# quartiq/stabilizer-stream

Hardware: NVIDIA B200
Metric: sustained MS/s through full PSD cascade (higher is better)
Workload: dtype f32

## Files before the change

stabilizer_stream_b200/csrc/sspsd_cascade.cu:

```cuda
#if defined(__x86_64__)
#include <emmintrin.h>
#endif

#include "sspsd_cascade.cuh"

#include <algorithm>
#include <cmath>
#include <cstdlib>
#include <cstring>
#include <mutex>

#include "sspsd_decim_kernel.cuh"
#include "sspsd_stage_kernel.cuh"
#include "sspsd_stage_kernel_r16.cuh"
#include "sspsd_stage_kernel_ring.cuh"
#include "sspsd_stage_kernel_w16.cuh"

namespace sspsd {

static thread_local std::string g_err;
void set_error(const std::string& msg) { g_err = msg; }
const char* last_error() { return g_err.c_str(); }

bool cuda_ok(cudaError_t e, const char* what)
{
    if (e == cudaSuccess)
        return true;
    set_error(std::string(what) + ": " + cudaGetErrorString(e));
    return false;
}

namespace {

inline long long floor4(long long v) { return v & ~3ll; }

template <int LOG2N>
int launch_stage_t(const StageParams& p, int grid, cudaStream_t s)
{
    size_t smem = stage_smem_bytes<LOG2N>(p.T, p.hop);
    psd_stage_kernel<LOG2N><<<grid, Plan<LOG2N>::NT, smem, s>>>(p);
    return cuda_ok(cudaGetLastError(), "psd_stage_kernel launch") ? SSPSD_OK : SSPSD_ECUDA;
}

template <int LOG2N>
int prepare_stage_t(int hop, int budget_bytes, int* tmax)
{
    using PL = Plan<LOG2N>;
    int t = 256;
    while (t > 1 && (long long)stage_smem_bytes<LOG2N>(t, hop) > budget_bytes)
        --t;
    if ((long long)stage_smem_bytes<LOG2N>(t, hop) > budget_bytes) {
        set_error("FFT size does not fit in shared memory");
        return SSPSD_EINVAL;
    }
    *tmax = t;
    (void)PL::N;
    if (!cuda_ok(cudaFuncSetAttribute(psd_stage_kernel<LOG2N>, cudaFuncAttributeMaxDynamicSharedMemorySize,
// ... 27 lines not shown
    default:
        return SSPSD_EINVAL;
    }
}

int prepare_stage(int log2n, bool r16, int hop, int* tmax, int* nt)
{
    if (log2n == 12 && r16) {
        int t = 64;
        while (t > 1 && (long long)stage_r16_smem_bytes(t, hop) > 112 * 1024) --t;
        *tmax = t;
        *nt = R16::NT;
        SSPSD_CUDA(cudaFuncSetAttribute(psd_stage_kernel_r16, cudaFuncAttributeMaxDynamicSharedMemorySize,
                                        (int)stage_r16_smem_bytes(t, hop)));
        SSPSD_CUDA(cudaFuncSetAttribute(psd_stage_kernel_ring, cudaFuncAttributeMaxDynamicSharedMemorySize,
                                        (int)stage_ring_smem_bytes(RingCfg::MAX_W)));
        SSPSD_CUDA(cudaFuncSetAttribute(psd_stage_kernel_ring1, cudaFuncAttributeMaxDynamicSharedMemorySize,
                                        (int)stage_ring_smem_bytes(1024, 1, RingCfg::RING1, false)));
        SSPSD_CUDA(cudaFuncSetAttribute(psd_stage_kernel_ring1x5, cudaFuncAttributeMaxDynamicSharedMemorySize,
                                        (int)stage_ring_smem_bytes(384, 1, 3, false)));
        return SSPSD_OK;
    }
    if (log2n == 9)
        SSPSD_CUDA(cudaFuncSetAttribute(psd_stage_kernel_w16, cudaFuncAttributeMaxDynamicSharedMemorySize,
                                        (int)stage_w16_smem_bytes(W16::MAX_T)));
    switch (log2n) {
#define X(L)                                                                   \
    case L:                                                                    \
        *nt = Plan<L>::NT;                                                     \
        return prepare_stage_t<L>(hop, Plan<L>::NT <= 256 ? 100 * 1024 : 200 * 1024, tmax);
        SSPSD_FOR_SIZES(X)
#undef X
    default:
        set_error("n_fft must be a power of two in 64..8192");
        return SSPSD_EINVAL;
    }
}

template <int MA, int MB, int MC, int PRESET>
int launch_decim_t(const DecimParams& p, int grid, cudaStream_t s)
{
    using GE = DecGeom<MA, MB, MC>;
    decim8_kernel<MA, MB, MC, PRESET><<<grid, DEC_NT, GE::SMEM_FLOATS * sizeof(float), s>>>(p);
    return cuda_ok(cudaGetLastError(), "decim8_kernel launch") ? SSPSD_OK : SSPSD_ECUDA;
}

template <int MA, int MB, int MC, int PRESET, int OB, int CTAS>
int launch_decim_tma_t(const DecimParams& p, long long n_out, int num_sms, cudaStream_t s)
{
    const int ntiles = (int)((n_out + OB - 1) / OB);
    const int grid = std::min(ntiles, num_sms * CTAS);
    decim8_tma_kernel<MA, MB, MC, PRESET, OB, CTAS><<<grid, DEC_NT, decim_tma_smem_bytes<MA, MB, MC, OB>(), s>>>(p, ntiles);
    return cuda_ok(cudaGetLastError(), "decim8_tma_kernel launch") ? SSPSD_OK : SSPSD_ECUDA;
}

template <int MA, int MB, int MC, int PRESET, int OB, int CTAS>
int launch_decim_async_t(const DecimParams& p, long long n_out, int num_sms, cudaStream_t s)
{
    const int ntiles = (int)((n_out + OB - 1) / OB);
    const int grid = std::min(ntiles, num_sms * CTAS);
    decim8_async_kernel<MA, MB, MC, PRESET, OB, CTAS><<<grid, DEC_NT, decim_async_smem_bytes<MA, MB, MC, OB>(), s>>>(p, ntiles);
    return cuda_ok(cudaGetLastError(), "decim8_async_kernel launch") ? SSPSD_OK : SSPSD_ECUDA;
}

template <int MA, int MB, int MC, int PRESET, int OB, int CTAS>
int launch_decim_pf_t(const DecimParams& p, long long n_out, int num_sms, cudaStream_t s)
{
    const int ntiles = (int)((n_out + OB - 1) / OB);
    const int grid = std::min(ntiles, num_sms * CTAS);
    decim8_pf_kernel<MA, MB, MC, PRESET, OB, CTAS><<<grid, DEC_NT, decim_pf_smem_bytes<MA, MB, MC, OB>(), s>>>(p, ntiles);
    return cuda_ok(cudaGetLastError(), "decim8_pf_kernel launch") ? SSPSD_OK : SSPSD_ECUDA;
}

int decim_halo(int preset)
{
    return preset == SSPSD_HBF_98 ? DecGeom<3, 6, 15>::HALO : DecGeom<5, 10, 23>::HALO;
}

int upload_taps_once(int device)
{
    static std::mutex mu;
    static bool done[64] = {false};
    std::lock_guard<std::mutex> lock(mu);
    if (device < 64 && done[device])
        return SSPSD_OK;
    static_assert(sizeof(sspsd_hbf_taps) == sizeof(float) * SSPSD_HBF_NPRESET * 3 * SSPSD_HBF_MAXTAPS, "tap table");
    {
        float t0[SSPSD_HBF_NPRESET][3][SSPSD_HBF_MAXTAPS + 1], t1[SSPSD_HBF_NPRESET][3][SSPSD_HBF_MAXTAPS + 1];
        for (int p = 0; p < SSPSD_HBF_NPRESET; ++p)
            for (int s = 0; s < 3; ++s)
                for (int i = 0; i <= SSPSD_HBF_MAXTAPS; ++i) {
                    t0[p][s][i] = i < SSPSD_HBF_MAXTAPS ? sspsd_hbf_taps[p][s][i] : 0.f;
                    t1[p][s][i] = i + 1 < SSPSD_HBF_MAXTAPS ? sspsd_hbf_taps[p][s][i + 1] : 0.f;
                }
        SSPSD_CUDA(cudaMemcpyToSymbol(c_hbf_taps, t0, sizeof(t0)));
        SSPSD_CUDA(cudaMemcpyToSymbol(c_hbf_taps_sh, t1, sizeof(t1)));
    }
    SSPSD_CUDA(cudaFuncSetAttribute(decim8_kernel<5, 10, 23, SSPSD_HBF_140>, cudaFuncAttributeMaxDynamicSharedMemorySize,
                                    (int)(DecGeom<5, 10, 23>::SMEM_FLOATS * sizeof(float))));
    SSPSD_CUDA(cudaFuncSetAttribute(decim8_kernel<3, 6, 15, SSPSD_HBF_98>, cudaFuncAttributeMaxDynamicSharedMemorySize,
                                    (int)(DecGeom<3, 6, 15>::SMEM_FLOATS * sizeof(float))));
    SSPSD_CUDA(cudaFuncSetAttribute(decim8_async_kernel<5, 10, 23, SSPSD_HBF_140, 960, 2>,
                                    cudaFuncAttributeMaxDynamicSharedMemorySize, (int)decim_async_smem_bytes<5, 10, 23, 960>()));
    SSPSD_CUDA(cudaFuncSetAttribute(decim8_async_kernel<5, 10, 23, SSPSD_HBF_140, 640, 3>,
                                    cudaFuncAttributeMaxDynamicSharedMemorySize, (int)decim_async_smem_bytes<5, 10, 23, 640>()));
    SSPSD_CUDA(cudaFuncSetAttribute(decim8_async_kernel<3, 6, 15, SSPSD_HBF_98, 960, 2>,
                                    cudaFuncAttributeMaxDynamicSharedMemorySize, (int)decim_async_smem_bytes<3, 6, 15, 960>()));
    SSPSD_CUDA(cudaFuncSetAttribute(decim8_async_kernel<3, 6, 15, SSPSD_HBF_98, 640, 3>,
                                    cudaFuncAttributeMaxDynamicSharedMemorySize, (int)decim_async_smem_bytes<3, 6, 15, 640>()));
    SSPSD_CUDA(cudaFuncSetAttribute(decim8_tma_kernel<5, 10, 23, SSPSD_HBF_140, 960, 2>,
                                    cudaFuncAttributeMaxDynamicSharedMemorySize, (int)decim_tma_smem_bytes<5, 10, 23, 960>()));
    SSPSD_CUDA(cudaFuncSetAttribute(decim8_tma_kernel<5, 10, 23, SSPSD_HBF_140, 640, 3>,
                                    cudaFuncAttributeMaxDynamicSharedMemorySize, (int)decim_tma_smem_bytes<5, 10, 23, 640>()));
    SSPSD_CUDA(cudaFuncSetAttribute(decim8_tma_kernel<3, 6, 15, SSPSD_HBF_98, 960, 2>,
                                    cudaFuncAttributeMaxDynamicSharedMemorySize, (int)decim_tma_smem_bytes<3, 6, 15, 960>()));
    SSPSD_CUDA(cudaFuncSetAttribute(decim8_tma_kernel<3, 6, 15, SSPSD_HBF_98, 640, 3>,
                                    cudaFuncAttributeMaxDynamicSharedMemorySize, (int)decim_tma_smem_bytes<3, 6, 15, 640>()));
    SSPSD_CUDA(cudaFuncSetAttribute(decim8_tma_kernel<5, 10, 23, SSPSD_HBF_140, 768, 3>,
                                    cudaFuncAttributeMaxDynamicSharedMemorySize, (int)decim_tma_smem_bytes<5, 10, 23, 768>()));
    SSPSD_CUDA(cudaFuncSetAttribute(decim8_tma_kernel<3, 6, 15, SSPSD_HBF_98, 768, 3>,
                                    cudaFuncAttributeMaxDynamicSharedMemorySize, (int)decim_tma_smem_bytes<3, 6, 15, 768>()));
    SSPSD_CUDA(cudaFuncSetAttribute(decim8_pf_kernel<5, 10, 23, SSPSD_HBF_140, 960, 2>,
                                    cudaFuncAttributeMaxDynamicSharedMemorySize, (int)decim_pf_smem_bytes<5, 10, 23, 960>()));
    SSPSD_CUDA(cudaFuncSetAttribute(decim8_pf_kernel<5, 10, 23, SSPSD_HBF_140, 640, 3>,
                                    cudaFuncAttributeMaxDynamicSharedMemorySize, (int)decim_pf_smem_bytes<5, 10, 23, 640>()));
    SSPSD_CUDA(cudaFuncSetAttribute(decim8_pf_kernel<3, 6, 15, SSPSD_HBF_98, 960, 2>,
                                    cudaFuncAttributeMaxDynamicSharedMemorySize, (int)decim_pf_smem_bytes<3, 6, 15, 960>()));
    SSPSD_CUDA(cudaFuncSetAttribute(decim8_pf_kernel<3, 6, 15, SSPSD_HBF_98, 640, 3>,
                                    cudaFuncAttributeMaxDynamicSharedMemorySize, (int)decim_pf_smem_bytes<3, 6, 15, 640>()));
    if (device < 64)
        done[device] = true;
    return SSPSD_OK;
}

struct EwmaPlan {
    int jb;
    float g_first;
    float g_s;
    float total;
    uint32_t count_after;
};

EwmaPlan ewma_plan(uint32_t count, uint32_t avg, uint64_t S)
{
    EwmaPlan e{};
    uint32_t steady = avg + 1u;
    e.g_s = (float)avg / (float)steady;
    uint64_t jb;
    if (count > avg) {
        jb = 0;
        e.g_first = (float)avg / (float)count;
    } else {
        jb = (uint64_t)avg - count + 1;
        e.g_first = e.g_s;
    }
    if (jb >= S) {
        e.jb = (int)S;
        e.total = 1.0f;
        e.count_after = (uint32_t)(count + S);
    } else {
        e.jb = (int)jb;
        double t = (double)e.g_first;
        uint64_t n_s = S - 1 - jb;
        if (n_s > 0)
            t *= std::pow((double)e.g_s, (double)n_s);
        e.total = (float)t;
        e.count_after = steady;
    }
    return e;
}

}

int hbf_info(int hbf, uint32_t* drain, uint32_t* halo)
// ... 81 lines not shown
    std::vector<float> win(n);
    if (cfg.window == SSPSD_WINDOW_RECT) {
        std::fill(win.begin(), win.end(), 1.0f);
        win_ = {1.0f, 1.0f, 0};
    } else {
        const float pi = 3.14159265358979323846f;
        float df = pi / (float)n;
        for (uint32_t i = 0; i < n; ++i) {
            float s = sinf(df * (float)i);
            win[i] = s * s;
        }
        win_ = {0.25f, 1.5f, n / 2};
    }
    hop_ = n - win_.overlap;
    drain_ = sspsd_hbf_drain[cfg.hbf];
    int halo = decim_halo(cfg.hbf);
    hb_ = std::max<int>((int)win_.overlap, halo);
    hb_ = (hb_ + 7) & ~7;

    SSPSD_CUDA(cudaDeviceGetAttribute(&num_sms_, cudaDevAttrMultiProcessorCount, cfg.device));
    if (cfg.stream) {
        stream_ = (cudaStream_t)cfg.stream;
    } else {
        SSPSD_CUDA(cudaStreamCreateWithFlags(&stream_, cudaStreamNonBlocking));
        own_stream_ = true;
    }
    SSPSD_CUDA(cudaStreamCreateWithFlags(&copy_stream_, cudaStreamNonBlocking));
    const char* ov = getenv("SSPSD_OVERLAP");
    deep_from_ = ov ? (size_t)atoi(ov) : 1;
    if (max_stages_ > 1 && deep_from_ > 0 && !one_stream_) {
        int lo_prio = 0, hi_prio = 0;
        SSPSD_CUDA(cudaDeviceGetStreamPriorityRange(&lo_prio, &hi_prio));
        SSPSD_CUDA(cudaStreamCreateWithPriority(&deep_stream_, cudaStreamNonBlocking, hi_prio));
        SSPSD_CUDA(cudaEventCreateWithFlags(&ev_stage0_, cudaEventDisableTiming));
        SSPSD_CUDA(cudaEventCreateWithFlags(&ev_deep_, cudaEventDisableTiming));
        const char* ps = getenv("SSPSD_PSD_STREAM");
        if (!ps || atoi(ps) != 0) {
            SSPSD_CUDA(cudaStreamCreateWithPriority(&psd_stream_, cudaStreamNonBlocking, hi_prio));
            SSPSD_CUDA(cudaEventCreateWithFlags(&ev_psd_join_, cudaEventDisableTiming));
        }
    }
    for (int i = 0; i < 2; ++i) {
        SSPSD_CUDA(cudaEventCreateWithFlags(&ev_copied_[i], cudaEventDisableTiming));
        SSPSD_CUDA(cudaEventCreateWithFlags(&ev_free_[i], cudaEventDisableTiming));
        SSPSD_CUDA(cudaEventCreateWithFlags(&ev_stage_[i], cudaEventDisableTiming));
    }
    int rc = upload_taps_once(cfg.device);
    if (rc) return rc;
    defer_ = cfg_.deep_defer ? cfg_.deep_defer : (1ull << 26);
    if (const char* e = getenv("SSPSD_DEFER")) defer_ = strtoull(e, nullptr, 0);
    k2_variant_ = k2_variant_from_env();
    {
        const char* e = getenv("SSPSD_K3");
        std::string m = e ? e : "tma960";
        k3_variant_ = m == "tiled" ? 0 : m == "tma960" ? 1 : m == "tma640" ? 2 : m == "async640" ? 4 : m == "pf960" ? 5 :
                      m == "pf640" ? 6 : m == "tma768" ? 7 : 3;
    }
    rc = prepare_stage((int)log2n_, k2_variant_ >= 1, (int)hop_, &tmax_, &nt_);
    if (rc) return rc;

    const uint32_t m = n / 2;
    std::vector<float2> twM(m), twN(m);
    for (uint32_t k = 0; k < m; ++k) {
        double a = -2.0 * M_PI * (double)k / (double)m;
        twM[k] = make_float2((float)std::cos(a), (float)std::sin(a));
        double b = -2.0 * M_PI * (double)k / (double)n;
        twN[k] = make_float2((float)std::cos(b), (float)std::sin(b));
    }
    acc_stride_ = (m + 1 + 63) & ~63u;
    SSPSD_CUDA(cudaMalloc(&d_win_, n * sizeof(float)));
    SSPSD_CUDA(cudaMalloc(&d_twM_, m * sizeof(float2)));
    SSPSD_CUDA(cudaMalloc(&d_twN_, m * sizeof(float2)));
    SSPSD_CUDA(cudaMalloc(&d_acc_, (size_t)SSPSD_MAX_STAGES * acc_stride_ * sizeof(float)));
    SSPSD_CUDA(cudaMemcpyAsync(d_win_, win.data(), n * sizeof(float), cudaMemcpyHostToDevice, stream_));
    SSPSD_CUDA(cudaMemcpyAsync(d_twM_, twM.data(), m * sizeof(float2), cudaMemcpyHostToDevice, stream_));
    SSPSD_CUDA(cudaMemcpyAsync(d_twN_, twN.data(), m * sizeof(float2), cudaMemcpyHostToDevice, stream_));
    SSPSD_CUDA(cudaMemsetAsync(d_acc_, 0, (size_t)SSPSD_MAX_STAGES * acc_stride_ * sizeof(float), stream_));
    SSPSD_CUDA(cudaMallocHost(&h_acc_, (size_t)SSPSD_MAX_STAGES * acc_stride_ * sizeof(float)));
    SSPSD_CUDA(cudaStreamSynchronize(stream_));
    stages_.reserve(SSPSD_MAX_STAGES);
    n_ = n;
    return SSPSD_OK;
}

uint32_t Cascade::stage_avg(size_t i) const
{
    unsigned sh = (unsigned)(SSPSD_DEPTH * i);
    uint32_t v = sh >= 32 ? 0u : (avg_.count >> sh);
    return std::min(v, avg_.limit);
}

int Cascade::add_stage()
{
    if (stages_.size() >= SSPSD_MAX_STAGES) {
        set_error("too many stages");
        return SSPSD_EINVAL;
    }
    StageState st;
    const size_t cap = (size_t)hb_ + n_ + 16;
    cudaStream_t ss = stage_stream(stages_.size());
    if (!spare_.empty()) {
        StageState old = spare_.back();
        spare_.pop_back();
        st.carry[0] = old.carry[0];
        st.carry[1] = old.carry[1];
        st.fresh[0] = old.fresh[0];
        st.fresh[1] = old.fresh[1];
        st.fresh_cap = old.fresh_cap;
        st.ev_read[0] = old.ev_read[0];
// ... 149 lines not shown
    rc = launch_stage((int)log2n_, k2_variant_ >= 1, p, grid, psd_stream(i));
    prof_end(psd_stream(i));
    if (rc) return rc;
    return reduce_partials(i, grid * groups, p);
}

int Cascade::prepare_partials(size_t i, int rows, StageParams* p)
{
    p->part = nullptr;
    p->part_stride = 0;
    if (!(cfg_.flags & SSPSD_FLAG_DETERMINISTIC)) return SSPSD_OK;
    const int which = psd_stream(i) == stream_ ? 0 : 1;
    const size_t need = (size_t)rows * acc_stride_;
    if (need > part_cap_[which]) {
        SSPSD_CUDA(cudaStreamSynchronize(psd_stream(i)));
        if (d_part_[which]) SSPSD_CUDA(cudaFree(d_part_[which]));
        d_part_[which] = nullptr;
        SSPSD_CUDA(cudaMalloc(&d_part_[which], need * sizeof(float)));
        part_cap_[which] = need;
    }
    p->part = d_part_[which];
    p->part_stride = (int)acc_stride_;
    return SSPSD_OK;
}

int Cascade::reduce_partials(size_t i, int rows, const StageParams& p)
{
    if (!p.part) return SSPSD_OK;
    const int nb = (int)(n_ / 2 + 1);
    prof_begin(SSPSD_PROF_OTHER, 0, psd_stream(i));
    reduce_partials_kernel<<<(nb + 127) / 128, 128, 0, psd_stream(i)>>>(p.acc, p.part, rows, p.part_stride, nb);
    prof_end(psd_stream(i));
    return cuda_ok(cudaGetLastError(), "reduce_partials_kernel launch") ? SSPSD_OK : SSPSD_ECUDA;
}

int Cascade::launch_decim(size_t i, const StreamSrc& src, uint64_t m0, uint64_t m1, float* out_fresh,
                          long long out_split, long long out_cap)
{
    DecimParams p{};
    p.src = src;
    p.m0 = (long long)m0;
    p.m1 = (long long)m1;
    p.drain = drain_;
    p.out_fresh = out_fresh;
    p.out_split = out_split;
    p.out_cap = out_cap;
    p.preset = cfg_.hbf;
    long long lo = std::max<long long>(p.m0, p.drain);
    if (p.m1 <= lo)
        return SSPSD_OK;
    int grid = (int)((p.m1 - lo + DEC_OB - 1) / DEC_OB);
    cudaStream_t ss = stage_stream(i);
    static const bool fuse_carry = !getenv("SSPSD_CARRY_KERNEL");
    if (cc_valid_ && fuse_carry && (k3_variant_ == 1 || k3_variant_ == 2 || k3_variant_ == 7)) {
        p.cc = cc_pending_;
        cc_valid_ = false;
    }
    prof_begin(i == 0 ? SSPSD_PROF_DECIM_STAGE0 : SSPSD_PROF_DECIM_DEEP, (uint64_t)(p.m1 - lo) * 8, ss);
    int rc;
    if (k3_variant_ == 0) {
        rc = cfg_.hbf == SSPSD_HBF_98 ? launch_decim_t<3, 6, 15, SSPSD_HBF_98>(p, grid, ss)
                                      : launch_decim_t<5, 10, 23, SSPSD_HBF_140>(p, grid, ss);
    } else if (k3_variant_ == 1) {
        rc = cfg_.hbf == SSPSD_HBF_98 ? launch_decim_tma_t<3, 6, 15, SSPSD_HBF_98, 960, 2>(p, p.m1 - lo, num_sms_, ss)
                                      : launch_decim_tma_t<5, 10, 23, SSPSD_HBF_140, 960, 2>(p, p.m1 - lo, num_sms_, ss);
    } else if (k3_variant_ == 2) {
        rc = cfg_.hbf == SSPSD_HBF_98 ? launch_decim_tma_t<3, 6, 15, SSPSD_HBF_98, 640, 3>(p, p.m1 - lo, num_sms_, ss)
                                      : launch_decim_tma_t<5, 10, 23, SSPSD_HBF_140, 640, 3>(p, p.m1 - lo, num_sms_, ss);
    } else if (k3_variant_ == 3) {
        rc = cfg_.hbf == SSPSD_HBF_98 ? launch_decim_async_t<3, 6, 15, SSPSD_HBF_98, 960, 2>(p, p.m1 - lo, num_sms_, ss)
                                      : launch_decim_async_t<5, 10, 23, SSPSD_HBF_140, 960, 2>(p, p.m1 - lo, num_sms_, ss);
    } else if (k3_variant_ == 7) {
        rc = cfg_.hbf == SSPSD_HBF_98 ? launch_decim_tma_t<3, 6, 15, SSPSD_HBF_98, 768, 3>(p, p.m1 - lo, num_sms_, ss)
                                      : launch_decim_tma_t<5, 10, 23, SSPSD_HBF_140, 768, 3>(p, p.m1 - lo, num_sms_, ss);
    } else if (k3_variant_ == 5) {
        rc = cfg_.hbf == SSPSD_HBF_98 ? launch_decim_pf_t<3, 6, 15, SSPSD_HBF_98, 960, 2>(p, p.m1 - lo, num_sms_, ss)
                                      : launch_decim_pf_t<5, 10, 23, SSPSD_HBF_140, 960, 2>(p, p.m1 - lo, num_sms_, ss);
    } else if (k3_variant_ == 6) {
        rc = cfg_.hbf == SSPSD_HBF_98 ? launch_decim_pf_t<3, 6, 15, SSPSD_HBF_98, 640, 3>(p, p.m1 - lo, num_sms_, ss)
                                      : launch_decim_pf_t<5, 10, 23, SSPSD_HBF_140, 640, 3>(p, p.m1 - lo, num_sms_, ss);
    } else {
        rc = cfg_.hbf == SSPSD_HBF_98 ? launch_decim_async_t<3, 6, 15, SSPSD_HBF_98, 640, 3>(p, p.m1 - lo, num_sms_, ss)
                                      : launch_decim_async_t<5, 10, 23, SSPSD_HBF_140, 640, 3>(p, p.m1 - lo, num_sms_, ss);
    }
    prof_end(ss);
    return rc;
}

int Cascade::run_stage(size_t i, const float* fresh, long long split, uint64_t n_new)
{
    StageState& st = stages_[i];
    cudaStream_t ss = stage_stream(i);
    cudaStream_t ps = psd_stream(i);
    const uint64_t L1 = st.L + n_new;
    const uint64_t craw0 = st.craw;
    const uint64_t craw1 = L1 < n_ ? 0 : 1 + (L1 - n_) / hop_;
    const StreamSrc src{st.carry[st.cur], fresh, st.carry_start, split, (long long)L1};
    int rc;
    bool psd_launched = false;
    if (ps != ss && craw1 > craw0) {
        SSPSD_CUDA(cudaEventRecord(st.ev_in, ss));
        SSPSD_CUDA(cudaStreamWaitEvent(ps, st.ev_in, 0));
    }

    if (windowed_ && i < n_local_ && craw1 > craw0) {
        const uint64_t step = (uint64_t)hop_ << (SSPSD_DEPTH * i);
        const uint64_t c = own_offset(i);
        auto first_at_or_after = [&](uint64_t pos) { return pos <= c ? 0ull : (pos - c + step - 1) / step; };
        uint64_t klo = std::max<uint64_t>(first_at_or_after(own_lo_), (st.valid_from + hop_ - 1) / hop_);
        uint64_t khi = own_hi_ == ~0ull ? ~0ull : first_at_or_after(own_hi_);
        uint64_t a = std::max(craw0, klo), b = std::min(craw1, khi);
        if (b > a) {
            if (st.avg == 0xffffffffu) {
// ... 958 lines not shown
```

stabilizer_stream_b200/csrc/sspsd_cascade.cuh:

```cuda
#pragma once
#include <cuda_runtime.h>

#include <cstdint>
#include <string>
#include <vector>

#include "../../include/sspsd.h"
#include "sspsd_device.cuh"

namespace sspsd {

struct StageParams;
void set_error(const std::string& msg);
const char* last_error();
int hbf_info(int hbf, uint32_t* drain, uint32_t* halo);
bool cuda_ok(cudaError_t e, const char* what);

struct DeviceGuard {
    int prev = -1;
    bool ok = true;
    explicit DeviceGuard(int dev)
    {
        if (cudaGetDevice(&prev) != cudaSuccess) prev = -1;
        ok = prev == dev || cuda_ok(cudaSetDevice(dev), "cudaSetDevice");
// ... 98 lines not shown
    cudaStream_t stage_stream(size_t i) const { return (i < deep_from_ || !deep_stream_) ? stream_ : deep_stream_; }
    cudaStream_t psd_stream(size_t i) const { return (i >= deep_from_ && psd_stream_) ? psd_stream_ : stage_stream(i); }
    int join_streams();
    uint64_t defer_threshold(size_t j) const;
    int run_pending(size_t j);
    int flush_deferred();
    int ensure_fresh(StageState& st, size_t need, size_t reserve = 0);
    int ensure_in_buffers(size_t need);
    int process_host(const float* x, size_t n);
    int flush_staged();
    int feed_device_chunk(const float* x, size_t n);
    int feed_host_chunk(const float* xh, size_t n);
    static uint64_t host_chunk() { return 1ull << 23; }
    float gain_of(uint32_t count) const;
    uint32_t stage_avg(size_t i) const;
    uint64_t decimated(const StageState& st) const { return st.craw ? n_ + (st.craw - 1) * (uint64_t)hop_ : 0; }

    struct ProfRec {
        int cls;
        cudaEvent_t a, b;
        uint64_t units;
    };
    bool prof_on_ = false;
    std::vector<ProfRec> prof_;
    uint64_t launches_[SSPSD_PROF_NCLASS] = {0, 0, 0, 0, 0};
    void prof_begin(int cls, uint64_t units, cudaStream_t s);
    void prof_end(cudaStream_t s);

    bool windowed_ = false;
    uint64_t own_lo_ = 0, own_hi_ = ~0ull;
    uint32_t n_local_ = SSPSD_MAX_STAGES;
    float* d_tail_ = nullptr;
    size_t tail_cap_ = 0, tail_len_ = 0;
    uint64_t tail_first_ = 0;
    uint64_t seek_pos_ = 0;
    uint64_t next_valid_from(uint64_t valid) const;
    uint64_t own_offset(size_t i) const;

    StageHook* hook_ = nullptr;
    bool one_stream_ = false;
    sspsd_config cfg_{};
    uint32_t n_ = 0, log2n_ = 0, hop_ = 0, max_stages_ = SSPSD_MAX_STAGES;
    WindowInfo win_{};
    int detrend_ = 0;
    sspsd_avg_opts avg_{0xffffffffu, 0xffffffffu};
    int hb_ = 0;
    int drain_ = 0;
    int num_sms_ = 148;
    int tmax_ = 1, nt_ = 256;
    uint64_t defer_ = 1ull << 26;
    uint64_t defer_window_ = 0;
    CarryJob cc_pending_{};
    bool cc_valid_ = false;
    int k3_variant_ = 1;
    int k2_variant_ = 2;
    bool single_stage_avg_set_ = false;
    uint32_t single_stage_avg_ = 0xffffffffu;
    cudaStream_t stream_ = nullptr;
    bool own_stream_ = false;
    cudaStream_t copy_stream_ = nullptr;
    cudaStream_t deep_stream_ = nullptr;
    cudaStream_t psd_stream_ = nullptr;
    cudaEvent_t ev_stage0_ = nullptr, ev_deep_ = nullptr, ev_psd_join_ = nullptr;
    bool deep_dirty_ = false, psd_dirty_ = false;
    size_t deep_from_ = 1;
    cudaEvent_t ev_copied_[2] = {nullptr, nullptr}, ev_free_[2] = {nullptr, nullptr};
    cudaEvent_t ev_stage_[2] = {nullptr, nullptr};
    int last_copy_ = -1;
    std::vector<StageState> stages_;
    std::vector<StageState> spare_;
    float* d_win_ = nullptr;
    float2* d_twM_ = nullptr;
    float2* d_twN_ = nullptr;
    float* d_acc_ = nullptr;
    uint32_t acc_stride_ = 0;
    float* h_stage_[2] = {nullptr, nullptr};
    int stage_buf_ = 0;
    bool stage_pending_[2] = {false, false};
    size_t staged_ = 0;
    float* d_in_[2] = {nullptr, nullptr};
    size_t d_in_cap_ = 0;
    int in_buf_ = 0;
    float* h_acc_ = nullptr;
    float* d_part_[2] = {nullptr, nullptr};
    size_t part_cap_[2] = {0, 0};
    float* d_sink_ = nullptr;
    size_t sink_cap_ = 0, sink_len_ = 0;
};

}

struct sspsd_cascade {
    sspsd::Cascade c;
};
struct sspsd_stage {
    sspsd::Cascade c;
};
```

stabilizer_stream_b200/csrc/sspsd_decim_kernel.cuh:

```cuda
#pragma once
#include "sspsd_device.cuh"
#include "sspsd_hbf_taps.h"

namespace sspsd {

__constant__ __align__(8) float c_hbf_taps[SSPSD_HBF_NPRESET][3][SSPSD_HBF_MAXTAPS + 1];
__constant__ __align__(8) float c_hbf_taps_sh[SSPSD_HBF_NPRESET][3][SSPSD_HBF_MAXTAPS + 1];

constexpr int DEC_OB = 960;
constexpr int DEC_P = 8;
constexpr int DEC_LP = 3;
constexpr int DEC_NT = 256;

constexpr int roundup(int v, int m) { return (v + m - 1) / m * m; }

template <int MA, int MB, int MC, int OB_ = DEC_OB>
struct DecGeom {
    static constexpr int OB = OB_;
    static constexpr int NB = roundup(2 * OB + 4 * MC - 2, DEC_P);
    static constexpr int NA = roundup(2 * NB + 4 * MB - 2, DEC_P);
    static constexpr int NX = roundup(2 * NA + 4 * MA - 2, 8);
    static constexpr int HALO = NX - 8 * OB;
    static constexpr int phase_stride(int len) { return ((len + DEC_P - 1) / DEC_P + 27) / 32 * 32 + 4; }
    static constexpr int SX = phase_stride(NX / 2), SA = phase_stride(NA / 2), SB = phase_stride(NB / 2);
    static constexpr int SMEM_FLOATS = 2 * DEC_P * (SX + SA + SB);
};

__device__ __forceinline__ void carry_job(const StreamSrc& src, const CarryJob& c)
{
    SSPSD_ASSERT(c.n >= 0 && c.n <= c.dst_cap && c.head_n >= 0 && c.head_n < 4);
    for (int i = blockIdx.x * blockDim.x + threadIdx.x; i < c.n; i += gridDim.x * blockDim.x) {
        const float v = ld_stream1(src, c.g0 + i);
        c.dst[i] = v;
        if (i >= c.n - c.head_n) c.head_dst[i - (c.n - c.head_n)] = v;
    }
}

struct DecimParams {
    CarryJob cc;
    StreamSrc src;
    long long m0, m1;
    long long drain;
    float* out_fresh;
    long long out_split;
    long long out_cap;
    int preset;
};

template <int M, int SI, int SO, int REL0, bool FINAL, int PRESET, int SET>
__device__ __forceinline__ void hbf_stage(const float* __restrict__ ine, const float* __restrict__ ino,
                                          int n_out, float* __restrict__ oute,
                                          float* __restrict__ outo, float* __restrict__ gout, int rel_lo, int rel_hi,
                                          long long gidx0 = 0, long long gcap = 0)
{
    (void)gidx0;
    (void)gcap;
    constexpr int P = DEC_P, LP = DEC_LP;
    for (int w = threadIdx.x; w < n_out / P; w += DEC_NT) {
        constexpr int NW = 2 * M + P - 1;
        float2 wp[(NW + 1) / 2];
#pragma unroll
        for (int i = 0; i < NW; ++i) {
            const int c = REL0 - 2 * M + 1 + i;
            const float x = ino[(c & (P - 1)) * SI + (c >> LP) + w];
            if (i & 1) wp[i >> 1].y = x; else wp[i >> 1].x = x;
        }
        const float2* __restrict__ tp0 = reinterpret_cast<const float2*>(&c_hbf_taps[PRESET][SET][0]);
        const float2* __restrict__ tp1 = reinterpret_cast<const float2*>(&c_hbf_taps_sh[PRESET][SET][0]);
        float y[P];
#pragma unroll
        for (int q = 0; q < P; ++q) {
            float2 acc = make_float2(0.f, 0.f);
            constexpr int dummy = 0;
            (void)dummy;
            const int i0 = q & 1;
#pragma unroll
            for (int i = i0; i + 1 < M; i += 2) {
                const float2 l = wp[(q + i) >> 1];
                const float2 r = wp[(q + 2 * M - 2 - i) >> 1];
                const float2 sum = __fadd2_rn(l, make_float2(r.y, r.x));
                acc = __ffma2_rn(sum, (q & 1) ? tp1[(i - 1) >> 1] : tp0[i >> 1], acc);
            }
            float a = acc.x + acc.y;
            auto winv = [&](int k) { return (k & 1) ? wp[k >> 1].y : wp[k >> 1].x; };
            if (q & 1) a = fmaf(winv(q) + winv(q + 2 * M - 1), c_hbf_taps[PRESET][SET][0], a);
            if (((M - i0) & 1) != 0) a = fmaf(winv(q + M - 1) + winv(q + M), c_hbf_taps[PRESET][SET][M - 1], a);
            const int ce = REL0 + q - M + 1;
            y[q] = ine[(ce & (P - 1)) * SI + (ce >> LP) + w] + a;
        }
        if constexpr (FINAL) {
#pragma unroll
            for (int q = 0; q < P; ++q) {
                const int r = P * w + q;
                if (r >= rel_lo && r < rel_hi) {
                    SSPSD_ASSERT(gidx0 + r >= 0 && gidx0 + r < gcap);
                    gout[r] = y[q];
                }
            }
        } else {
            const int pb = (w & 1) * (P / 2) * SO + (w >> 1);
#pragma unroll
            for (int r = 0; r < P / 2; ++r) {
                oute[pb + r * SO] = y[2 * r];
                outo[pb + r * SO] = y[2 * r + 1];
            }
        }
    }
}

template <int MA, int MB, int MC, int PRESET>
__global__ void __launch_bounds__(DEC_NT) decim8_kernel(const DecimParams p)
{
    using GE = DecGeom<MA, MB, MC>;
    extern __shared__ __align__(16) float smem[];
    float* xe = smem;
    float* xo = xe + DEC_P * GE::SX;
    float* ae = xo + DEC_P * GE::SX;
    float* ao = ae + DEC_P * GE::SA;
    float* be = ao + DEC_P * GE::SA;
    float* bo = be + DEC_P * GE::SB;

    const long long mhi = p.m1 - (long long)blockIdx.x * DEC_OB;
    const long long x_base = 8 * mhi - GE::NX;
    const long long c_base = mhi - DEC_OB;

    if (x_base >= p.src.split) {
        const float4* __restrict__ gx = reinterpret_cast<const float4*>(p.src.fresh + (x_base - p.src.split));
        constexpr int NV = GE::NX / 4;
#pragma unroll 2
        for (int v0 = 0; v0 < NV; v0 += 4 * DEC_NT) {
            float4 f[4];
#pragma unroll
            for (int u = 0; u < 4; ++u) {
                const int v = v0 + u * DEC_NT + threadIdx.x;
                if (v < NV) f[u] = __ldg(gx + v);
            }
#pragma unroll
            for (int u = 0; u < 4; ++u) {
                const int v = v0 + u * DEC_NT + threadIdx.x;
// ... 196 lines not shown
            if (v < NV) {
                const int pos = 2 * (v & 3) * GE::SX + (v >> 2);
                xe[pos] = pf[u].x;
                xo[pos] = pf[u].y;
                xe[pos + GE::SX] = pf[u].z;
                xo[pos + GE::SX] = pf[u].w;
            }
        }
    };
    int tile = blockIdx.x;
    if (tile < ntiles) {
        fetch(tile);
        scatter();
    }
    const long long lo = p.m0 > p.drain ? p.m0 : p.drain;
    for (; tile < ntiles; tile += gridDim.x) {
        const long long mhi = p.m1 - (long long)tile * OB;
        const long long c_base = mhi - OB;
        const int next = tile + (int)gridDim.x;
        __syncthreads();
        if (next < ntiles) fetch(next);
        hbf_stage<MA, GE::SX, GE::SA, GE::NX / 2 - GE::NA, false, PRESET, 2>(xe, xo, GE::NA, ae, ao, nullptr, 0, 0);
        __syncthreads();
        hbf_stage<MB, GE::SA, GE::SB, GE::NA / 2 - GE::NB, false, PRESET, 1>(ae, ao, GE::NB, be, bo, nullptr, 0, 0);
        __syncthreads();
        if (next < ntiles) scatter();
        const int rel_lo = lo > c_base ? (int)(lo - c_base) : 0;
        hbf_stage<MC, GE::SB, GE::SB, GE::NB / 2 - OB, true, PRESET, 0>(be, bo, OB, nullptr, nullptr,
                                                                        p.out_fresh + (c_base - p.drain - p.out_split),
                                                                        rel_lo, OB, c_base - p.drain - p.out_split, p.out_cap);
    }
}

template <int MA, int MB, int MC, int OB>
constexpr size_t decim_pf_smem_bytes()
{
    return (size_t)DecGeom<MA, MB, MC, OB>::SMEM_FLOATS * sizeof(float);
}

template <int MA, int MB, int MC, int OB>
constexpr size_t decim_async_smem_bytes()
{
    using GE = DecGeom<MA, MB, MC, OB>;
    return (size_t)(2 * (2 * DEC_P * GE::SX + 4) + 2 * DEC_P * (GE::SA + GE::SB)) * sizeof(float);
}

template <int MA, int MB, int MC, int OB>
constexpr size_t decim_tma_smem_bytes()
{
    using GE = DecGeom<MA, MB, MC, OB>;
    return (size_t)(GE::NX + GE::SMEM_FLOATS) * sizeof(float) + 16;
}

__global__ void carry_copy_kernel(StreamSrc src, long long g0, int n, float* __restrict__ dst,
                                  float* __restrict__ head_dst, int head_n, int dst_cap)
{
    carry_job(src, CarryJob{g0, n, head_n, dst, head_dst, dst_cap});
}

__global__ void scale_kernel(float* __restrict__ acc, int n, float s)
{
    int i = blockIdx.x * blockDim.x + threadIdx.x;
    if (i < n)
        acc[i] *= s;
}

}
```

stabilizer_stream_b200/csrc/sspsd_device.cuh:

```cuda
#pragma once
#include <cuda_runtime.h>
#include <stdint.h>

#ifdef SSPSD_BOUNDS
#include <assert.h>
#define SSPSD_ASSERT(c) assert(c)
#else
#define SSPSD_ASSERT(c) ((void)0)
#endif

namespace sspsd {

struct StreamSrc {
    const float* carry;
    const float* fresh;
    long long carry_start;
    long long split;
    long long end;
};

struct CarryJob {
    long long g0;
    int n, head_n;
    float* dst;
// ... 1 lines not shown
    int dst_cap;
};

__device__ __forceinline__ float4 ld_stream4(const StreamSrc& s, long long g)
{
    SSPSD_ASSERT(g + 4 <= s.end && (g & 3) == 0);
    if (g >= s.split)
        return __ldg(reinterpret_cast<const float4*>(s.fresh + (g - s.split)));
    if (g >= s.carry_start)
        return *reinterpret_cast<const float4*>(s.carry + (g - s.carry_start));
    return make_float4(0.f, 0.f, 0.f, 0.f);
}

__device__ __forceinline__ float ld_stream1(const StreamSrc& s, long long g)
{
    SSPSD_ASSERT(g < s.end);
    if (g >= s.split)
        return __ldg(s.fresh + (g - s.split));
    if (g >= s.carry_start)
        return s.carry[g - s.carry_start];
    return 0.f;
}

__device__ __forceinline__ uint32_t smem_u32(const void* p) { return (uint32_t)__cvta_generic_to_shared(p); }

__device__ __forceinline__ void mbar_init(uint64_t* bar, uint32_t count)
{
    asm volatile("mbarrier.init.shared::cta.b64 [%0], %1;" ::"r"(smem_u32(bar)), "r"(count) : "memory");
}
__device__ __forceinline__ void mbar_expect_tx(uint64_t* bar, uint32_t bytes)
{
    asm volatile("mbarrier.arrive.expect_tx.shared::cta.b64 _, [%0], %1;" ::"r"(smem_u32(bar)), "r"(bytes) : "memory");
}
__device__ __forceinline__ void mbar_wait(uint64_t* bar, uint32_t parity)
{
    asm volatile(
        "{\n\t"
        ".reg .pred p;\n\t"
        "WAIT_%=:\n\t"
        "mbarrier.try_wait.parity.shared::cta.b64 p, [%0], %1;\n\t"
        "@p bra DONE_%=;\n\t"
        "bra WAIT_%=;\n\t"
        "DONE_%=:\n\t"
        "}" ::"r"(smem_u32(bar)),
        "r"(parity)
        : "memory");
}
__device__ __forceinline__ void bulk_g2s(void* dst, const void* src, uint32_t bytes, uint64_t* bar)
{
    asm volatile("cp.async.bulk.shared::cluster.global.mbarrier::complete_tx::bytes [%0], [%1], %2, [%3];" ::"r"(
                     smem_u32(dst)),
                 "l"(src), "r"(bytes), "r"(smem_u32(bar))
                 : "memory");
}

__device__ __forceinline__ void ring_issue(const StreamSrc& s, long long g, int n, float* dst, uint64_t* bar)
{
    SSPSD_ASSERT(n >= 0 && (n & 3) == 0 && (g & 3) == 0 && (n == 0 || (g >= s.carry_start && g + n <= s.end)));
    mbar_expect_tx(bar, (uint32_t)n * 4u);
    long long nc = s.split - g;
    if (nc > n) nc = n;
    if (nc > 0) {
        bulk_g2s(dst, s.carry + (g - s.carry_start), (uint32_t)nc * 4u, bar);
    } else {
        nc = 0;
    }
    if (nc < n) bulk_g2s(dst + nc, s.fresh + (g + nc - s.split), (uint32_t)(n - nc) * 4u, bar);
}

template <int LOG2N>
struct Plan {
    static constexpr int N = 1 << LOG2N;
    static constexpr int LOG2M = LOG2N - 1;
    static constexpr int M = 1 << LOG2M;
    static constexpr int TPS = M / 8;
    static constexpr int NT = TPS > 256 ? TPS : 256;
    static constexpr int G = NT / TPS;
    static constexpr int REM = LOG2M - 2;
    static constexpr int A = REM / 3;
    static constexpr int EXTRA = REM % 3;
    static constexpr int P = A + (EXTRA ? 1 : 0) + 1;
    static constexpr int K = M / 4;
    static constexpr int WS = M + 4 * (M / 32);
    static_assert(LOG2N >= 6 && LOG2N <= 13, "supported FFT sizes: 64..8192");
    static_assert(A >= 1, "first pass must be radix 8");

    __host__ __device__ static constexpr int log2radix(int p) { return p < A ? 3 : (p == P - 1 ? 2 : EXTRA); }
    __host__ __device__ static constexpr int log2stride(int p)
    {
        int s = LOG2M;
        for (int q = 0; q <= p; ++q) s -= log2radix(q);
        return s;
    }
    __host__ __device__ static constexpr int log2weight(int p)
    {
        int s = 0;
        for (int q = 0; q < p; ++q) s += log2radix(q);
        return s;
    }
};

__device__ __forceinline__ int ws_pos(int i) { return i + ((i >> 5) << 2); }

__device__ __forceinline__ float2 cadd(float2 a, float2 b) { return __fadd2_rn(a, b); }
__device__ __forceinline__ float2 csub(float2 a, float2 b) { return __fadd2_rn(a, make_float2(-b.x, -b.y)); }
__device__ __forceinline__ float2 cadd_mi(float2 a, float2 b) { return __fadd2_rn(a, make_float2(b.y, -b.x)); }
// ... 86 lines not shown
```

Measured before the change: 240,500.

## Add tensor-map TMA decimation kernel with swizzled tile loads as default

```diff
diff --git a/stabilizer_stream_b200/csrc/sspsd_cascade.cu b/stabilizer_stream_b200/csrc/sspsd_cascade.cu
--- a/stabilizer_stream_b200/csrc/sspsd_cascade.cu
+++ b/stabilizer_stream_b200/csrc/sspsd_cascade.cu
@@ -3,6 +3,8 @@
 #endif
 
 #include "sspsd_cascade.cuh"
+
+#include <cudaTypedefs.h>
 
 #include <algorithm>
 #include <cmath>
@@ -136,6 +138,52 @@
     const int grid = std::min(ntiles, num_sms * CTAS);
     decim8_tma_kernel<MA, MB, MC, PRESET, OB, CTAS><<<grid, DEC_NT, decim_tma_smem_bytes<MA, MB, MC, OB>(), s>>>(p, ntiles);
     return cuda_ok(cudaGetLastError(), "decim8_tma_kernel launch") ? SSPSD_OK : SSPSD_ECUDA;
+}
+
+PFN_cuTensorMapEncodeTiled_v12000 tensor_map_encoder()
+{
+    static PFN_cuTensorMapEncodeTiled_v12000 fn = [] {
+        void* f = nullptr;
+        cudaDriverEntryPointQueryResult q{};
+        if (cudaGetDriverEntryPointByVersion("cuTensorMapEncodeTiled", &f, 12000, cudaEnableDefault, &q) != cudaSuccess ||
+            q != cudaDriverEntryPointSuccess)
+            f = nullptr;
+        return reinterpret_cast<PFN_cuTensorMapEncodeTiled_v12000>(f);
+    }();
+    return fn;
+}
+
+template <int MA, int MB, int MC, int PRESET, int OB, int CTAS>
+int launch_decim_tmap_t(const DecimParams& p, long long n_out, int num_sms, cudaStream_t s)
+{
+    using GT = DecTmapGeom<MA, MB, MC, OB>;
+    const int ntiles = (int)((n_out + OB - 1) / OB);
+    const int grid = std::min(ntiles, num_sms * CTAS);
+    const long long off = ((8 * p.m1 - GT::NX - p.src.split) % 32 + 32) % 32;
+    const long long rows = std::min<long long>((p.src.end - p.src.split - off) / 32, 1ll << 30);
+    CUtensorMap map{};
+    int map_rows = 0;
+    if (rows >= GT::ROWS) {
+        PFN_cuTensorMapEncodeTiled_v12000 encode = tensor_map_encoder();
+        if (!encode) {
+            set_error("cuTensorMapEncodeTiled is not available from the driver");
+            return SSPSD_ECUDA;
+        }
+        const cuuint64_t dim[2] = {32, (cuuint64_t)rows};
+        const cuuint64_t stride[1] = {32 * sizeof(float)};
+        const cuuint32_t box[2] = {32, GT::ROWS}, estride[2] = {1, 1};
+        const CUresult r = encode(&map, CU_TENSOR_MAP_DATA_TYPE_FLOAT32, 2, const_cast<float*>(p.src.fresh + off), dim, stride,
+                                  box, estride, CU_TENSOR_MAP_INTERLEAVE_NONE, CU_TENSOR_MAP_SWIZZLE_128B,
+                                  CU_TENSOR_MAP_L2_PROMOTION_L2_256B, CU_TENSOR_MAP_FLOAT_OOB_FILL_NONE);
+        if (r != CUDA_SUCCESS) {
+            set_error("cuTensorMapEncodeTiled failed: " + std::to_string((int)r));
+            return SSPSD_ECUDA;
+        }
+        map_rows = (int)rows;
+    }
+    decim8_tmap_kernel<MA, MB, MC, PRESET, OB, CTAS>
+        <<<grid, DEC_NT, GT::SMEM_BYTES, s>>>(p, ntiles, map, p.src.split + off, map_rows);
+    return cuda_ok(cudaGetLastError(), "decim8_tmap_kernel launch") ? SSPSD_OK : SSPSD_ECUDA;
 }
 
 template <int MA, int MB, int MC, int PRESET, int OB, int CTAS>
@@ -204,6 +252,10 @@
                                     cudaFuncAttributeMaxDynamicSharedMemorySize, (int)decim_tma_smem_bytes<5, 10, 23, 768>()));
     SSPSD_CUDA(cudaFuncSetAttribute(decim8_tma_kernel<3, 6, 15, SSPSD_HBF_98, 768, 3>,
                                     cudaFuncAttributeMaxDynamicSharedMemorySize, (int)decim_tma_smem_bytes<3, 6, 15, 768>()));
+    SSPSD_CUDA(cudaFuncSetAttribute(decim8_tmap_kernel<5, 10, 23, SSPSD_HBF_140, 960, 3>,
+                                    cudaFuncAttributeMaxDynamicSharedMemorySize, (int)DecTmapGeom<5, 10, 23, 960>::SMEM_BYTES));
+    SSPSD_CUDA(cudaFuncSetAttribute(decim8_tmap_kernel<3, 6, 15, SSPSD_HBF_98, 960, 3>,
+                                    cudaFuncAttributeMaxDynamicSharedMemorySize, (int)DecTmapGeom<3, 6, 15, 960>::SMEM_BYTES));
     SSPSD_CUDA(cudaFuncSetAttribute(decim8_pf_kernel<5, 10, 23, SSPSD_HBF_140, 960, 2>,
                                     cudaFuncAttributeMaxDynamicSharedMemorySize, (int)decim_pf_smem_bytes<5, 10, 23, 960>()));
     SSPSD_CUDA(cudaFuncSetAttribute(decim8_pf_kernel<5, 10, 23, SSPSD_HBF_140, 640, 3>,
@@ -391,9 +443,9 @@
     k2_variant_ = k2_variant_from_env();
     {
         const char* e = getenv("SSPSD_K3");
-        std::string m = e ? e : "tma960";
+        std::string m = e ? e : "tmap960";
         k3_variant_ = m == "tiled" ? 0 : m == "tma960" ? 1 : m == "tma640" ? 2 : m == "async640" ? 4 : m == "pf960" ? 5 :
-                      m == "pf640" ? 6 : m == "tma768" ? 7 : 3;
+                      m == "pf640" ? 6 : m == "tma768" ? 7 : m == "async960" ? 3 : 8;
     }
     rc = prepare_stage((int)log2n_, k2_variant_ >= 1, (int)hop_, &tmax_, &nt_);
     if (rc) return rc;
@@ -649,13 +701,16 @@
     int grid = (int)((p.m1 - lo + DEC_OB - 1) / DEC_OB);
     cudaStream_t ss = stage_stream(i);
     static const bool fuse_carry = !getenv("SSPSD_CARRY_KERNEL");
-    if (cc_valid_ && fuse_carry && (k3_variant_ == 1 || k3_variant_ == 2 || k3_variant_ == 7)) {
+    if (cc_valid_ && fuse_carry && (k3_variant_ == 1 || k3_variant_ == 2 || k3_variant_ == 7 || k3_variant_ == 8)) {
         p.cc = cc_pending_;
         cc_valid_ = false;
     }
     prof_begin(i == 0 ? SSPSD_PROF_DECIM_STAGE0 : SSPSD_PROF_DECIM_DEEP, (uint64_t)(p.m1 - lo) * 8, ss);
     int rc;
-    if (k3_variant_ == 0) {
+    if (k3_variant_ == 8) {
+        rc = cfg_.hbf == SSPSD_HBF_98 ? launch_decim_tmap_t<3, 6, 15, SSPSD_HBF_98, 960, 3>(p, p.m1 - lo, num_sms_, ss)
+                                      : launch_decim_tmap_t<5, 10, 23, SSPSD_HBF_140, 960, 3>(p, p.m1 - lo, num_sms_, ss);
+    } else if (k3_variant_ == 0) {
         rc = cfg_.hbf == SSPSD_HBF_98 ? launch_decim_t<3, 6, 15, SSPSD_HBF_98>(p, grid, ss)
                                       : launch_decim_t<5, 10, 23, SSPSD_HBF_140>(p, grid, ss);
     } else if (k3_variant_ == 1) {
diff --git a/stabilizer_stream_b200/csrc/sspsd_cascade.cuh b/stabilizer_stream_b200/csrc/sspsd_cascade.cuh
--- a/stabilizer_stream_b200/csrc/sspsd_cascade.cuh
+++ b/stabilizer_stream_b200/csrc/sspsd_cascade.cuh
@@ -174,7 +174,7 @@
     uint64_t defer_window_ = 0;
     CarryJob cc_pending_{};
     bool cc_valid_ = false;
-    int k3_variant_ = 1;
+    int k3_variant_ = 8;
     int k2_variant_ = 2;
     bool single_stage_avg_set_ = false;
     uint32_t single_stage_avg_ = 0xffffffffu;
diff --git a/stabilizer_stream_b200/csrc/sspsd_decim_kernel.cuh b/stabilizer_stream_b200/csrc/sspsd_decim_kernel.cuh
--- a/stabilizer_stream_b200/csrc/sspsd_decim_kernel.cuh
+++ b/stabilizer_stream_b200/csrc/sspsd_decim_kernel.cuh
@@ -1,4 +1,6 @@
 #pragma once
+#include <cuda.h>
+
 #include "sspsd_device.cuh"
 #include "sspsd_hbf_taps.h"
 
@@ -47,6 +49,27 @@
     int preset;
 };
 
+template <int M, int PRESET, int SET, int NWP>
+__device__ __forceinline__ float hbf_tap_sum(const float2 (&wp)[NWP], const int q)
+{
+    const float2* __restrict__ tp0 = reinterpret_cast<const float2*>(&c_hbf_taps[PRESET][SET][0]);
+    const float2* __restrict__ tp1 = reinterpret_cast<const float2*>(&c_hbf_taps_sh[PRESET][SET][0]);
+    float2 acc = make_float2(0.f, 0.f);
+    const int i0 = q & 1;
+#pragma unroll
+    for (int i = i0; i + 1 < M; i += 2) {
+        const float2 l = wp[(q + i) >> 1];
+        const float2 r = wp[(q + 2 * M - 2 - i) >> 1];
+        const float2 sum = __fadd2_rn(l, make_float2(r.y, r.x));
+        acc = __ffma2_rn(sum, (q & 1) ? tp1[(i - 1) >> 1] : tp0[i >> 1], acc);
+    }
+    float a = acc.x + acc.y;
+    auto winv = [&](int k) { return (k & 1) ? wp[k >> 1].y : wp[k >> 1].x; };
+    if (q & 1) a = fmaf(winv(q) + winv(q + 2 * M - 1), c_hbf_taps[PRESET][SET][0], a);
+    if (((M - i0) & 1) != 0) a = fmaf(winv(q + M - 1) + winv(q + M), c_hbf_taps[PRESET][SET][M - 1], a);
+    return a;
+}
+
 template <int M, int SI, int SO, int REL0, bool FINAL, int PRESET, int SET>
 __device__ __forceinline__ void hbf_stage(const float* __restrict__ ine, const float* __restrict__ ino,
                                           int n_out, float* __restrict__ oute,
@@ -65,26 +88,10 @@
             const float x = ino[(c & (P - 1)) * SI + (c >> LP) + w];
             if (i & 1) wp[i >> 1].y = x; else wp[i >> 1].x = x;
         }
-        const float2* __restrict__ tp0 = reinterpret_cast<const float2*>(&c_hbf_taps[PRESET][SET][0]);
-        const float2* __restrict__ tp1 = reinterpret_cast<const float2*>(&c_hbf_taps_sh[PRESET][SET][0]);
         float y[P];
 #pragma unroll
         for (int q = 0; q < P; ++q) {
-            float2 acc = make_float2(0.f, 0.f);
-            constexpr int dummy = 0;
-            (void)dummy;
-            const int i0 = q & 1;
-#pragma unroll
-            for (int i = i0; i + 1 < M; i += 2) {
-                const float2 l = wp[(q + i) >> 1];
-                const float2 r = wp[(q + 2 * M - 2 - i) >> 1];
-                const float2 sum = __fadd2_rn(l, make_float2(r.y, r.x));
-                acc = __ffma2_rn(sum, (q & 1) ? tp1[(i - 1) >> 1] : tp0[i >> 1], acc);
-            }
-            float a = acc.x + acc.y;
-            auto winv = [&](int k) { return (k & 1) ? wp[k >> 1].y : wp[k >> 1].x; };
-            if (q & 1) a = fmaf(winv(q) + winv(q + 2 * M - 1), c_hbf_taps[PRESET][SET][0], a);
-            if (((M - i0) & 1) != 0) a = fmaf(winv(q + M - 1) + winv(q + M), c_hbf_taps[PRESET][SET][M - 1], a);
+            const float a = hbf_tap_sum<M, PRESET, SET>(wp, q);
             const int ce = REL0 + q - M + 1;
             y[q] = ine[(ce & (P - 1)) * SI + (ce >> LP) + w] + a;
         }
@@ -387,6 +394,118 @@
     return (size_t)(GE::NX + GE::SMEM_FLOATS) * sizeof(float) + 16;
 }
 
+constexpr int DEC_TQ = 16;
+
+template <int MA, int MB, int MC, int OB_>
+struct DecTmapGeom {
+    using GE = DecGeom<MA, MB, MC, OB_>;
+    static constexpr int NB = GE::NB;
+    static constexpr int NA = roundup(2 * NB + 4 * MB - 2, DEC_TQ);
+    static constexpr int NX = roundup(2 * NA + 4 * MA - 2, 32);
+    static constexpr int ROWS = NX / 32;
+    static constexpr int XS = roundup(NX, 256);
+    static constexpr int SA = GE::phase_stride(NA / 2), SB = GE::SB;
+    static constexpr int S0 = 2 * (NX / 2 - NA) - 4 * MA + 3;
+    static constexpr size_t SMEM_BYTES = 1024 + (size_t)(XS + 2 * DEC_P * (SA + SB)) * sizeof(float) + 16;
+    static_assert((8 * OB_) % 32 == 0, "tile starts of a launch must be congruent mod 32 (one tensor-map origin)");
+    static_assert(ROWS <= 256 && NA / DEC_TQ <= DEC_NT, "one box, one stage-A work item per thread");
+    static_assert(S0 >= 0 && S0 + 4 * MA + 28 < 64, "a thread's window lies in its own row and the next");
+};
+
+template <int M, int NA, int S0, int SO, int PRESET>
+__device__ __forceinline__ void hbf_stage_a_tile(const float* __restrict__ x, float* __restrict__ oute, float* __restrict__ outo)
+{
+    constexpr int Q = DEC_TQ;
+    constexpr int NW = 2 * M + Q - 1;
+    constexpr int C0 = S0 / 4, C1 = (S0 + 2 * (NW - 1)) / 4;
+    constexpr int B = S0 - 4 * C0;
+    const int w = threadIdx.x;
+    if (w >= NA / Q) return;
+    float xs[4 * (C1 - C0 + 1)];
+#pragma unroll
+    for (int c = C0; c <= C1; ++c) {
+        const int row = w + (c >> 3);
+        const float4 v = lds128(x + 32 * row + (((c & 7) ^ (row & 7)) << 2));
+        xs[4 * (c - C0)] = v.x;
+        xs[4 * (c - C0) + 1] = v.y;
+        xs[4 * (c - C0) + 2] = v.z;
+        xs[4 * (c - C0) + 3] = v.w;
+    }
+    float2 wp[(NW + 1) / 2];
+#pragma unroll
+    for (int m = 0; m < (NW + 1) / 2; ++m) wp[m] = make_float2(xs[B + 4 * m], 2 * m + 1 < NW ? xs[B + 4 * m + 2] : 0.f);
+    float y[Q];
+#pragma unroll
+    for (int q = 0; q < Q; ++q) y[q] = xs[B + 2 * q + 2 * M - 1] + hbf_tap_sum<M, PRESET, 2>(wp, q);
+#pragma unroll
+    for (int r = 0; r < Q / 2; ++r) {
+        oute[r * SO + w] = y[2 * r];
+        outo[r * SO + w] = y[2 * r + 1];
+    }
+}
+
+template <int MA, int MB, int MC, int PRESET, int OB, int CTAS>
+__global__ void __launch_bounds__(DEC_NT, CTAS)
+    decim8_tmap_kernel(const DecimParams p, const int ntiles, const __grid_constant__ CUtensorMap tmap, const long long map_g0,
+                       const int map_rows)
+{
+    using GT = DecTmapGeom<MA, MB, MC, OB>;
+    extern __shared__ __align__(16) float smem[];
+    float* x = smem + ((1024u - (smem_u32(smem) & 1023u)) & 1023u) / sizeof(float);
+    float* ae = x + GT::XS;
+    float* ao = ae + DEC_P * GT::SA;
+    float* be = ao + DEC_P * GT::SA;
+    float* bo = be + DEC_P * GT::SB;
+    uint64_t* bar = reinterpret_cast<uint64_t*>(bo + DEC_P * GT::SB);
+
+    const int tid = threadIdx.x;
+    if (tid == 0) {
+        mbar_init(bar, 1);
+        asm volatile("fence.mbarrier_init.release.cluster;" ::: "memory");
+    }
+    __syncthreads();
+    auto x0 = [&](int t) { return 8 * (p.m1 - (long long)t * OB) - GT::NX; };
+    auto by_map = [&](long long g) { return g >= map_g0 && ((g - map_g0) >> 5) + GT::ROWS <= map_rows; };
+    auto issue = [&](int t) {
+        const long long g = x0(t);
+        if (!by_map(g)) return;
+        SSPSD_ASSERT(((g - map_g0) & 31) == 0 && g + GT::NX <= p.src.end);
+        mbar_expect_tx(bar, GT::NX * 4u);
+        tensor_g2s_2d(x, &tmap, 0, (int)((g - map_g0) >> 5), bar);
+    };
+    int tile = blockIdx.x;
+    if (tid == 0 && tile < ntiles) issue(tile);
+    if (p.cc.n) carry_job(p.src, p.cc);
+    const long long lo = p.m0 > p.drain ? p.m0 : p.drain;
+    uint32_t phase = 0;
+    for (; tile < ntiles; tile += gridDim.x) {
+        const long long g = x0(tile);
+        if (by_map(g)) {
+            mbar_wait(bar, phase);
+            phase ^= 1u;
+        } else {
+            for (int v = tid; v < GT::NX / 4; v += DEC_NT) {
+                const int row = v >> 3;
+                SSPSD_ASSERT(row < GT::ROWS);
+                *reinterpret_cast<float4*>(x + 32 * row + (((v & 7) ^ (row & 7)) << 2)) = ld_stream4(p.src, g + 4ll * v);
+            }
+            asm volatile("fence.proxy.async.shared::cta;" ::: "memory");
+            __syncthreads();
+        }
+        hbf_stage_a_tile<MA, GT::NA, GT::S0, GT::SA, PRESET>(x, ae, ao);
+        __syncthreads();
+        if (tid == 0 && tile + (int)gridDim.x < ntiles) issue(tile + (int)gridDim.x);
+        const long long mhi = p.m1 - (long long)tile * OB;
+        const long long c_base = mhi - OB;
+        hbf_stage<MB, GT::SA, GT::SB, GT::NA / 2 - GT::NB, false, PRESET, 1>(ae, ao, GT::NB, be, bo, nullptr, 0, 0);
+        __syncthreads();
+        const int rel_lo = lo > c_base ? (int)(lo - c_base) : 0;
+        hbf_stage<MC, GT::SB, GT::SB, GT::NB / 2 - OB, true, PRESET, 0>(be, bo, OB, nullptr, nullptr,
+                                                                        p.out_fresh + (c_base - p.drain - p.out_split),
+                                                                        rel_lo, OB, c_base - p.drain - p.out_split, p.out_cap);
+    }
+}
+
 __global__ void carry_copy_kernel(StreamSrc src, long long g0, int n, float* __restrict__ dst,
                                   float* __restrict__ head_dst, int head_n, int dst_cap)
 {
diff --git a/stabilizer_stream_b200/csrc/sspsd_device.cuh b/stabilizer_stream_b200/csrc/sspsd_device.cuh
--- a/stabilizer_stream_b200/csrc/sspsd_device.cuh
+++ b/stabilizer_stream_b200/csrc/sspsd_device.cuh
@@ -77,6 +77,21 @@
                      smem_u32(dst)),
                  "l"(src), "r"(bytes), "r"(smem_u32(bar))
                  : "memory");
+}
+
+__device__ __forceinline__ void tensor_g2s_2d(void* dst, const void* tmap, int x, int y, uint64_t* bar)
+{
+    asm volatile("cp.async.bulk.tensor.2d.shared::cluster.global.mbarrier::complete_tx::bytes [%0], [%1, {%2, %3}], [%4];" ::"r"(
+                     smem_u32(dst)),
+                 "l"(tmap), "r"(x), "r"(y), "r"(smem_u32(bar))
+                 : "memory");
+}
+
+__device__ __forceinline__ float4 lds128(const float* p)
+{
+    float4 v;
+    asm volatile("ld.volatile.shared.v4.f32 {%0, %1, %2, %3}, [%4];" : "=f"(v.x), "=f"(v.y), "=f"(v.z), "=f"(v.w) : "r"(smem_u32(p)));
+    return v;
 }
 
 __device__ __forceinline__ void ring_issue(const StreamSrc& s, long long g, int n, float* dst, uint64_t* bar)
```

Result: faster. 247,500 (median of 6 runs) (+2.9%).
